# CTPLab/Tera-MIND

Hardware: AMD Instinct MI355X
Metric: denoising steps/sec on 64x64x(2 stains x 2 z) patches (interior patch-steps/s) (higher is better)
Workload: dtype f32; 1 GPU; configs[1]: b=32 images x 1 interior 64x64 patch (P=1, 128 padded + 32 collage patches/step), rna_slc=4, rna_num=229, stain=all, DDPM T=50 schedule, f32, mode A (pad+patchify -> UNet -> DDPM update); parallelism=dp1 (independent patch batches)

## Files before the change

include/teramind_hip.h:

```cpp
#ifndef TERAMIND_HIP_H
#define TERAMIND_HIP_H

#include <stddef.h>
#include <stdint.h>

#ifdef __cplusplus
extern "C" {
#endif

#define TM_ABI_VERSION 1

enum {
  TM_OK = 0,
  TM_ERR_ARG = -1,
  TM_ERR_STATE = -2,
  TM_ERR_KEY = -3,
  TM_ERR_HIP = -4,
  TM_ERR_WORKSPACE = -5
};

enum { TM_DTYPE_F32 = 0, TM_DTYPE_BF16 = 1, TM_DTYPE_F16 = 2 };
enum { TM_SAMPLE_DDPM = 0, TM_SAMPLE_DDIM = 1 };

typedef struct tm_config {
// ... 153 lines not shown
                    int64_t x_vol, int64_t y_pitch, int64_t y_depth, int64_t y_vol, const float* win_host, int n, float C1,
                    float C2, double* out, void* stream);

int tm_avgpool2_pad3(const void* src, int dtype, int V, int D, int H, int W, int64_t src_pitch, int64_t src_depth,
                     int64_t src_vol, void* dst, int64_t dst_pitch, int64_t dst_depth, int64_t dst_vol, void* stream);

typedef struct tm_prof_stats {
  uint64_t launches;
  double total_ms;
  double nominal_flops;
  double executed_flops;
  double alg_bytes;
} tm_prof_stats;
int tm_profile_enable(tm_model* m, int on);
int tm_profile_collect(tm_model* m, tm_prof_stats* out);


int tm_op_to_cb8(const void* x_ncdhw, void* y_cb8, int N, int C, int Z, int H, int W, void* stream);
int tm_op_from_cb8(const void* x_cb8, void* y_ncdhw, int N, int C, int Z, int H, int W, void* stream);

int tm_op_conv_mfma(const void* x_cb8, const void* w_host, const void* bias_host, void* y_cb8,
                    int N, int Cin, int Cout, int Z, int S, int ksize, int zmode, int up2,
                    int tile_variant, void* stream);
int tm_op_conv_mfma_res(const void* x_cb8, const void* w_host, const void* bias_host, void* y_cb8, const void* res_cb8,
                        int res_half, int N, int Cin, int Cout, int Z, int S, int ksize, int zmode, int up2,
                        int tile_variant, void* stream);

int tm_op_conv_zpair_fused_f32(const void* x_cb8, const void* w_host, const void* bias_host, const void* norm_w_host,
                               const void* scale_host, const void* shift_host, const void* res_cb8, void* a2_out,
                               void* h1_out, void* a2_sep_out, int N, int Cin, int Cout, int Z, int S, int per_image,
                               int tile_variant, void* stream);

int tm_op_conv_ups_pair_f32(const void* x_cb8, const void* w_host, const void* bias_host, void* y_cb8, int N, int Cin,
                            int Cout, int Z, int S, int tile_variant, void* stream);

int tm_op_conv_xquad_f32(const void* x_cb8, const void* w_host, const void* bias_host, void* y_cb8, const void* res_cb8,
                         int res_half, int N, int Cin, int Cout, int Z, int S, int tile_variant, void* stream);
int tm_op_conv_xquad_sched_f32(const void* x_cb8, const void* w_host, const void* bias_host, void* y_cb8, const void* res_cb8,
                               int res_half, int N, int Cin, int Cout, int Z, int S, int tile_variant, int sched, void* stream);
int tm_conv_xquad_lds_bytes(int half, int tw, int sched);
int tm_op_conv_pad1_time_sched_f32(const void* x_cb8, const void* w_host, const void* bias_host, void* y_cb8, int N, int Cin,
                                   int Cout, int S, int form, int tile_variant, int sched, int iters, float* ms_out, void* stream);
int tm_op_conv_xquad_split_f32(const void* x_cb8, const void* w_host, const void* bias_host, void* y_cb8, const void* res_cb8,
                               int res_half, int N, int Cin, int Cout, int Z, int S, int tile_variant, int sched, int ksplit,
                               void* stream);
int tm_conv_xquad_ksplit(int N, int Cin, int Cout, int S, int res_half);
int tm_op_conv_pad1_time_split_f32(const void* x_cb8, const void* w_host, const void* bias_host, void* y_cb8, int N, int Cin,
                                   int Cout, int S, int form, int tile_variant, int sched, int ksplit, int iters, float* ms_out,
                                   void* stream);

int tm_op_conv1_f32(const void* x_cb8, const void* w_host, const void* bias_host, void* y_cb8, const void* res_cb8,
                    const void* gate_cb8, int x_cbtot, int x_cb0, int gate_cbtot, int gate_cb0, int gate_half, int gelu,
                    int tile_variant, int N, int Cin, int Cout, int Z, int S, int* form_out, void* stream);
int tm_conv1_form(long vox, int ntile, int tile_variant);

int tm_conv_frag_addrs(int kernel, int half, int tw, int what, int wave, int p, int ky, int kx, int sub, int* out64);

int tm_op_conv27_bf16(const void* x_cb8, const void* w_host, const void* bias_host, void* y_cb8,
                      int N, int Cin, int Cout, int S, int dtype, int waves, const void* res_h16, void* y_h16,
                      int ups, int res_half, void* stream);
int tm_op_conv27_h16_z(const void* x_cb8, const void* w_host, const void* bias_host, void* y_cb8,
                       int N, int Cin, int Cout, int S, int dtype, int waves, const void* res_h16, void* y_h16,
                       int ups, int res_half, int Z, void* stream);

int tm_op_conv27_time(int N, int Cin, int Cout, int S, int dtype, int waves, int ups, int with_res, int fused,
                      int iters, float* ms_per_launch, void* stream);

int tm_op_conv27_fused(const void* x_cb8, const void* w_host, const void* bias_host, const void* norm_w_host,
                       const void* scale_host, const void* shift_host, void* a2_out, int N, int Cin, int Cout,
                       int S, int per_image, int dtype, int waves, void* stream);
int tm_op_conv27_fused_z(const void* x_cb8, const void* w_host, const void* bias_host, const void* norm_w_host,
                         const void* scale_host, const void* shift_host, void* a2_out, int N, int Cin, int Cout,
                         int S, int per_image, int dtype, int waves, int Z, void* stream);

int tm_op_conv1_bf16(const void* x_cb8, const void* w_host, const void* bias_host, void* y_cb8,
                     int N, int Cin, int Cout, int Z, int S, int gelu, int dtype, int waves, const void* res_h16,
                     const void* gate_h16, void* y_h16, void* stream);

int tm_op_conv1_h16_gate(const void* x_cb8, const void* w_host, const void* bias_host, void* y_cb8,
                         int N, int Cin, int Cout, int Z, int S, int gelu, int dtype, int waves, const void* res_h16,
                         const void* gate_h16, void* y_h16, int gate_half, int gate_cbtot, int gate_cb0, void* stream);

int tm_op_conv1_concat(const void* const* x_cb8, const int* cin, const int* collage, int nsrc, const void* w_host,
                       const void* bias_host, void* y_cb8, int N, int Cout, int Z, int S, int p1, int p2,
                       int dtype, int waves, void* stream);

int tm_op_prep_h16(const void* const* src_h16, const int* src_c, const int* collage, int nsrc, int N, int Z, int S,
                   int p1, int p2, int up2, const void* norm_w_dev, int c_real, int mod, const void* mod_scale,
                   const void* mod_shift, long mod_stride, int per_image, int act, int dtype, int variant,
                   void* out_h16, void* raw_h16, int iters, float* elapsed_ms, void* stream);

int tm_op_prep_f32(const void* const* src_cb8, const int* src_c, const int* collage, int nsrc, int N, int Z, int S,
                   int p1, int p2, int up2, const void* norm_w_dev, int c_real, int mod, const void* mod_scale,
                   const void* mod_shift, long mod_stride, int mod_half, int per_image, int act, int variant,
                   void* out_cb8, void* raw_cb8, int iters, float* elapsed_ms, void* stream);

int tm_op_prep_form(const void* const* src, const int* src_c, const int* collage, int nsrc, int N, int Z, int S,
                    int p1, int p2, int resample, int src_dtype, int out_dtype, const void* norm_w_dev, int c_real,
                    int mod, int mod_dtype, const void* mod_scale, const void* mod_shift, long mod_stride, int mod_half,
                    int per_image, int act, int variant, int pad_blocks, void* out, void* raw, int raw_dtype,
                    int iters, float* elapsed_ms, void* stream);

int tm_op_stem(const void* x, const void* w_host, const void* bias_host, void* y, int N, int Cin, int Cout, int Z, int S,
               int dtype, void* stream);
int tm_op_head(const void* x_cb8, const void* w_host, const void* bias_host, void* y, int N, int C, int Cout, int Z, int S,
               int dtype, void* stream);
// ... 93 lines not shown
```

tera-mind_amd/_lib.py:

```python
import ctypes as C
import os

_HERE = os.path.dirname(os.path.abspath(__file__))
LIB_PATH = os.environ.get("TM_LIB_PATH") or os.path.join(_HERE, "csrc", "libteramind_hip.so")

c_void_p, c_int, c_size_t, c_char_p, c_float = C.c_void_p, C.c_int, C.c_size_t, C.c_char_p, C.c_float
c_i64_p = C.POINTER(C.c_int64)


class TmConfig(C.Structure):
    _fields_ = [("patch_size", C.c_int32), ("rna_slc", C.c_int32), ("n_stain", C.c_int32),
                ("rna_num", C.c_int32), ("net_ch", C.c_int32), ("ch_mult", C.c_int32 * 4),
                ("embed_ch", C.c_int32), ("attn_res", C.c_int32), ("num_res_blocks", C.c_int32),
                ("vis_only", C.c_int32), ("dtype", C.c_int32)]


class TmStepCoefs(C.Structure):
    _fields_ = [("sqrt_recip_alphas_cumprod", c_float), ("sqrt_recipm1_alphas_cumprod", c_float),
                ("posterior_mean_coef1", c_float), ("posterior_mean_coef2", c_float),
                ("sigma", c_float), ("sqrt_alpha_bar_prev", c_float),
                ("sqrt_one_minus_alpha_bar_prev", c_float)]


class TmProfStats(C.Structure):
# ... 24 lines not shown
    "tm_unet_forward": (c_int, [c_void_p, c_void_p, c_void_p, c_void_p, c_int, c_int, c_int,
                                c_void_p, c_void_p, c_void_p, c_size_t, c_void_p]),
    "tm_rna_level0_bytes": (c_size_t, [c_void_p, c_int, c_int, c_int]),
    "tm_rna_level0": (c_int, [c_void_p, c_void_p, c_int, c_int, c_int, c_void_p, c_size_t, c_void_p, c_size_t, c_void_p]),
    "tm_unet_forward_level0": (c_int, [c_void_p] * 4 + [c_size_t] + [c_int] * 3 + [c_void_p] * 3 + [c_size_t, c_void_p]),
    "tm_rna_pyramid_bytes": (c_size_t, [c_void_p, c_int, c_int, c_int]),
    "tm_rna_pyramid": (c_int, [c_void_p, c_void_p, c_int, c_int, c_int, c_void_p, c_size_t, c_void_p]),
    "tm_unet_forward_rna": (c_int, [c_void_p, c_void_p, c_void_p, c_void_p, c_size_t, c_int, c_int, c_int,
                                    c_void_p, c_void_p, c_void_p, c_size_t, c_void_p]),
    "tm_sampler_step": (c_int, [C.POINTER(TmStepCoefs), c_void_p, c_void_p, c_void_p, c_void_p,
                                c_int, c_int, c_int, c_int, c_int, c_int, c_void_p]),
    "tm_pad_patchify": (c_int, [c_void_p, c_void_p, c_int, c_int, c_int, c_int, c_int, c_float, c_void_p]),
    "tm_gene_attn_workspace_bytes": (c_size_t, [c_void_p, c_int]),
    "tm_gene_attn": (c_int, [c_void_p, c_void_p, c_int, c_void_p, c_void_p, c_void_p, c_size_t, c_void_p]),
    "tm_gene_attn_readout_workspace_bytes": (c_size_t, [c_void_p, c_int, c_int]),
    "tm_gene_attn_readout": (c_int, [c_void_p, c_void_p, c_int, C.POINTER(C.c_int), c_int, c_void_p, c_void_p, c_void_p,
                                     c_size_t, c_void_p]),
    "tm_model_destroy": (c_int, [c_void_p]),
    "tm_gene_tile_dense": (c_int, [c_void_p, c_void_p, C.c_int64] + [c_int] * 6 + [c_void_p, c_void_p]),
    "tm_train_batch_images": (c_int, [c_void_p] + [c_int] * 5 + [c_void_p, c_void_p] + [c_int] * 4 + [c_void_p, c_void_p]),
    "tm_train_batch_genes": (c_int, [c_void_p, c_void_p, C.c_int64, c_void_p, c_void_p] + [c_int] * 4 + [c_void_p, c_void_p] +
                             [c_int] * 5 + [c_void_p, c_void_p]),
    "tm_blosc_decompress": (c_int, [c_void_p, c_size_t, c_void_p, c_size_t, C.POINTER(c_size_t)]),
    "tm_blosc_bound": (c_size_t, [c_size_t, c_int, c_int]),
    "tm_blosc_compress": (c_int, [c_void_p, c_size_t, c_int, c_int, c_void_p, c_size_t, c_void_p, c_void_p]),
    "tm_blosc_compress_tiles": (c_int, [c_void_p, c_int, C.c_int64] + [c_int] * 3 + [C.c_int64] * 2 + [c_void_p, c_void_p, c_int, c_void_p,
                                        C.c_int64, c_void_p, c_void_p]),
    "tm_blosc_frame_info": (c_int, [c_void_p, c_size_t, c_void_p]),
    "tm_blosc_decompress_dev": (c_int, [c_void_p, c_void_p, c_void_p, c_int, c_void_p, C.c_int64, c_void_p, c_void_p, c_void_p]),
    "tm_blosc_decompress_tiles": (c_int, [c_void_p, c_void_p, c_void_p, c_int, c_void_p, c_int] + [C.c_int64] * 3 + [c_void_p] * 3),
    "tm_u8_shrink2": (c_int, [c_void_p, c_int, c_int, C.c_int64, c_void_p, C.c_int64, c_void_p]),
    "tm_jpeg_encode_tiles": (c_int, [c_void_p, c_int, c_int, C.c_int64] + [c_int] * 3 + [c_void_p, C.c_int64] + [c_void_p] * 4),
    "tm_jpeg_tables": (c_int, [c_int, c_void_p, c_size_t, C.POINTER(c_size_t)]),
    "tm_rgb_compose": (c_int, [C.POINTER(c_void_p), c_i64_p, c_int, c_int, c_float, c_void_p] + [c_int] * 3 +
                       [c_void_p, C.c_int64, c_void_p]),
    "tm_jpeg_encode_tiles_rgb": (c_int, [C.POINTER(c_void_p), c_i64_p, c_int, c_int, c_float, c_void_p] + [c_int] * 6 +
                                 [c_void_p, C.c_int64] + [c_void_p] * 4),
    "tm_jpeg_tables_rgb": (c_int, [c_int, c_void_p, c_size_t, C.POINTER(c_size_t)]),
    "tm_heat_field": (c_int, [c_void_p] + [c_int] * 3 + [C.c_int64] * 2 + [c_int, c_int, c_float, c_int, c_int, C.POINTER(c_float),
                              c_int, c_void_p, C.c_int64, c_void_p]),
    "tm_heat_render": (c_int, [c_void_p, c_int, c_int, C.c_int64, c_int, c_float, c_float, c_void_p, c_int, c_int,
                               C.POINTER(c_void_p), c_i64_p, c_void_p, C.c_int64, c_void_p]),
    "tm_ssim_planes": (c_int, [c_void_p, c_void_p] + [c_int] * 4 + [C.c_int64] * 4 + [C.POINTER(c_float), c_int, c_float, c_float, c_void_p, c_void_p]),
    "tm_avgpool2_pad": (c_int, [c_void_p] + [c_int] * 4 + [C.c_int64] * 2 + [c_void_p] + [C.c_int64] * 2 + [c_void_p]),
    "tm_ssim_volumes": (c_int, [c_void_p, c_void_p] + [c_int] * 5 + [C.c_int64] * 6 + [C.POINTER(c_float), c_int, c_float, c_float, c_void_p, c_void_p]),
    "tm_avgpool2_pad3": (c_int, [c_void_p] + [c_int] * 5 + [C.c_int64] * 3 + [c_void_p] + [C.c_int64] * 3 + [c_void_p]),
    "tm_profile_enable": (c_int, [c_void_p, c_int]),
    "tm_profile_collect": (c_int, [c_void_p, C.POINTER(TmProfStats)]),
    "tm_op_to_cb8": (c_int, [c_void_p, c_void_p, c_int, c_int, c_int, c_int, c_int, c_void_p]),
    "tm_op_from_cb8": (c_int, [c_void_p, c_void_p, c_int, c_int, c_int, c_int, c_int, c_void_p]),
    "tm_op_conv_mfma": (c_int, [c_void_p, c_void_p, c_void_p, c_void_p] + [c_int] * 9 + [c_void_p]),
    "tm_op_conv_mfma_res": (c_int, [c_void_p, c_void_p, c_void_p, c_void_p, c_void_p] + [c_int] * 10 + [c_void_p]),
    "tm_op_conv1_f32": (c_int, [c_void_p] * 6 + [c_int] * 12 + [C.POINTER(c_int), c_void_p]),
    "tm_conv1_form": (c_int, [C.c_long, c_int, c_int]),
    "tm_conv_frag_addrs": (c_int, [c_int] * 9 + [c_void_p]),
    "tm_op_conv27_bf16": (c_int, [c_void_p, c_void_p, c_void_p, c_void_p] + [c_int] * 6 + [c_void_p] * 2 + [c_int] * 2 + [c_void_p]),
    "tm_op_conv27_fused": (c_int, [c_void_p] * 7 + [c_int] * 7 + [c_void_p]),
    "tm_op_conv27_h16_z": (c_int, [c_void_p, c_void_p, c_void_p, c_void_p] + [c_int] * 6 + [c_void_p] * 2 + [c_int] * 3 + [c_void_p]),
    "tm_op_conv27_fused_z": (c_int, [c_void_p] * 7 + [c_int] * 8 + [c_void_p]),
    "tm_op_conv_zpair_fused_f32": (c_int, [c_void_p] * 10 + [c_int] * 7 + [c_void_p]),
    "tm_op_conv_ups_pair_f32": (c_int, [c_void_p] * 4 + [c_int] * 6 + [c_void_p]),
    "tm_op_conv_xquad_f32": (c_int, [c_void_p] * 5 + [c_int] * 7 + [c_void_p]),
    "tm_op_conv_xquad_sched_f32": (c_int, [c_void_p] * 5 + [c_int] * 8 + [c_void_p]),
    "tm_conv_xquad_lds_bytes": (c_int, [c_int] * 3),
    "tm_op_conv_pad1_time_sched_f32": (c_int, [c_void_p] * 4 + [c_int] * 8 + [C.POINTER(c_float), c_void_p]),
    "tm_op_conv_xquad_split_f32": (c_int, [c_void_p] * 5 + [c_int] * 9 + [c_void_p]),
    "tm_conv_xquad_ksplit": (c_int, [c_int] * 5),
    "tm_op_conv_pad1_time_split_f32": (c_int, [c_void_p] * 4 + [c_int] * 9 + [C.POINTER(c_float), c_void_p]),
    "tm_op_conv27_time":(c_int, [c_int] * 10 + [c_void_p, c_void_p]),
    "tm_op_conv1_bf16": (c_int, [c_void_p, c_void_p, c_void_p, c_void_p] + [c_int] * 8 + [c_void_p] * 4),
    "tm_op_conv1_h16_gate": (c_int, [c_void_p, c_void_p, c_void_p, c_void_p] + [c_int] * 8 + [c_void_p] * 3 + [c_int] * 3 + [c_void_p]),
    "tm_op_conv1_concat": (c_int, [c_void_p, c_void_p, c_void_p, c_int, c_void_p, c_void_p, c_void_p] + [c_int] * 8 + [c_void_p]),
    "tm_op_prep_h16": (c_int, [c_void_p] * 3 + [c_int] * 7 + [c_void_p, c_int, c_int, c_void_p, c_void_p, C.c_long] +
                       [c_int] * 4 + [c_void_p, c_void_p, c_int, c_void_p, c_void_p]),
    "tm_op_prep_f32": (c_int, [c_void_p] * 3 + [c_int] * 7 + [c_void_p, c_int, c_int, c_void_p, c_void_p, C.c_long] +
                       [c_int] * 4 + [c_void_p, c_void_p, c_int, c_void_p, c_void_p]),
    "tm_op_prep_form": (c_int, [c_void_p] * 3 + [c_int] * 9 + [c_void_p, c_int, c_int, c_int, c_void_p, c_void_p, C.c_long] +
                        [c_int] * 5 + [c_void_p, c_void_p, c_int, c_int, c_void_p, c_void_p]),
    "tm_op_stem": (c_int, [c_void_p] * 4 + [c_int] * 6 + [c_void_p]),
    "tm_op_head": (c_int, [c_void_p] * 4 + [c_int] * 6 + [c_void_p]),
    "tm_op_time_embed": (c_int, [c_void_p] * 7 + [c_int] * 3 + [c_void_p]),
    "tm_op_emb_all": (c_int, [c_void_p] * 4 + [c_int] * 3 + [c_void_p]),
    "tm_op_prep_train": (c_int, [c_void_p] * 5 + [c_float, c_int, c_void_p] + [c_int] * 4 + [c_void_p]),
    "tm_op_prep_bwd": (c_int, [c_void_p] * 6 + [c_float, c_int] + [c_void_p] * 4 + [c_int] * 4 + [c_void_p]),
    "tm_op_prep_train_rng": (c_int, [c_void_p] * 4 + [C.c_uint64, C.c_uint, c_float, c_int, c_void_p] + [c_int] * 4 + [c_void_p]),
    "tm_op_prep_bwd_rng": (c_int, [c_void_p] * 5 + [C.c_uint64, C.c_uint, c_float, c_int] + [c_void_p] * 4 + [c_int] * 4 + [c_void_p]),
    "tm_op_dropout_mask": (c_int, [C.c_uint64, C.c_uint, c_float, c_void_p] + [c_int] * 4 + [c_void_p]),
    "tm_op_conv_dgrad": (c_int, [c_void_p, c_void_p, c_void_p] + [c_int] * 6 + [c_void_p]),
    "tm_op_conv_wgrad": (c_int, [c_void_p, c_void_p, c_void_p, c_void_p] + [c_int] * 6 + [c_void_p]),
    "tm_conv_pack_floats": (C.c_long, [c_int] * 5),
    "tm_op_conv_pack_dev": (c_int, [c_void_p, c_void_p] + [c_int] * 5 + [c_void_p]),
    "tm_op_conv_mfma_packed": (c_int, [c_void_p] * 4 + [c_int] * 6 + [c_void_p]),
    "tm_op_conv_dgrad_packed": (c_int, [c_void_p] * 3 + [c_int] * 6 + [c_void_p]),
    "tm_op_conv_wgrad_dev": (c_int, [c_void_p] * 4 + [c_int] * 7 + [c_void_p]),
    "tm_op_conv_wgrad_time": (c_int, [c_int] * 9 + [c_void_p, c_void_p]),
    "tm_op_ew": (c_int, [c_int] + [c_void_p] * 5 + [C.c_long, c_void_p]),
    "tm_op_gemm_f32": (c_int, [c_void_p] * 4 + [c_int] * 3 + [c_void_p] + [c_int] * 3 + [c_float, c_void_p]),
    "tm_op_rows": (c_int, [c_int] + [c_void_p] * 5 + [C.c_long, c_int, c_void_p]),
    "tm_op_resample": (c_int, [c_void_p, c_void_p] + [c_int] * 5 + [c_void_p]),
    "tm_op_sumsq": (c_int, [c_void_p, C.c_long, c_void_p, c_void_p]),
    "tm_op_adam": (c_int, [c_void_p] * 4 + [C.c_long] + [c_float] * 5 + [c_int, c_float, c_void_p]),
    "tm_op_rank_sum": (c_int, [c_void_p, c_void_p, c_int, C.c_long, c_void_p]),
    "tm_op_rank_sum_time": (c_int, [c_int, C.c_long, c_int, c_int, c_void_p, c_void_p]),
    "tm_op_modnorm": (c_int, [c_void_p] * 5 + [c_int] * 4 + [c_void_p]),
    "tm_op_modnorm_bwd": (c_int, [c_void_p] * 8 + [c_int] * 4 + [c_void_p]),
    "tm_op_window_attn_train": (c_int, [c_void_p] * 12 + [c_int] * 4 + [c_void_p]),
# ... 45 lines not shown
```

tera-mind_amd/csrc/tm_kernels.hip:

```cpp
#include "tm_conv_pair.h"

#include <stdlib.h>
#include <string.h>

#include <type_traits>

namespace tmk {

template <int NZI, int WM, int TW, bool UPS = false>
struct C3Geo {
  static constexpr int TW_ = TW;
  static constexpr int MV = 4 * WM * 32;
  static constexpr int TR = (MV / TW < TW) ? (MV / TW) : TW;
  static constexpr int NPB = MV / (TR * TW);
  static constexpr int HR = TR + 2, HC = TW + 2;
  static constexpr int XV = NPB * NZI * HR * HC;
  static constexpr int XPIECES = XV * 2;
  static constexpr int PX = (XPIECES + 255) / 256;
  static constexpr int TZ = UPS ? 4 : 9;
  static constexpr int NTAP = TZ * NZI;
  static constexpr int WFLOATS = NTAP * 512;
  static constexpr int WPIECES = WFLOATS / 4;
  static constexpr int PW = (WPIECES + 255) / 256;
  static constexpr int TAPS_TOTAL = (NZI == 1) ? 9 : 3 * TZ;
// ... 791 lines not shown
  for (int z = 0; z < 2; ++z)
#pragma unroll
    for (int par = 0; par < 2; ++par) {
      f32x16 o = acc[0][par] + acc[1 + z][par];
      asm volatile("" : "+v"(o));
#pragma unroll
      for (int g = 0; g < 4; ++g) {
        f32x4 v;
        v[0] = o[4 * g + 0] + bv[g][0];
        v[1] = o[4 * g + 1] + bv[g][1];
        v[2] = o[4 * g + 2] + bv[g][2];
        v[3] = o[4 * g + 3] + bv[g][3];
        if (a.flags & EPI_GELU) {
#pragma unroll
          for (int j = 0; j < 4; ++j) v[j] = gelu_tanh_hw(v[j]);
        }
        if (a.res) v = rv[z][par][g] + v;
        rv[z][par][g] = v;
        asm volatile("" : "+v"(rv[z][par][g]));
      }
    }
#pragma unroll
  for (int z = 0; z < 2; ++z)
#pragma unroll
    for (int par = 0; par < 2; ++par)
#pragma unroll
      for (int g = 0; g < 4; ++g) {
        const int cob = nt * 4 + g;
        const long uni = (long)cob * a.y_plane + z * (S * S * 8) + par * 16;
        if (cob < a.Cob && okv) *(f32x4*)(a.y + yl + uni) = rv[z][par][g];
      }
}

constexpr int XQ_ZERO_FLOATS = 4096;
__device__ float xq_zero_bias[XQ_ZERO_FLOATS];
__global__ __launch_bounds__(256) void xquad_split_reduce(const float* part, long part_stride, int ksplit, const float* bias, const float* res,
                                                          long res_nstride, float* y, long y_nstride, long per_n4, int plane4, long total4,
                                                          int flags) {
  const long i = (long)blockIdx.x * 256 + threadIdx.x;
  if (i >= total4) return;
  const long n = i / per_n4, rem = i - n * per_n4;
  const long off = n * y_nstride + rem * 4;
  f32x4 v = *(const f32x4*)(part + off);
  for (int k = 1; k < ksplit; ++k) v = v + *(const f32x4*)(part + k * part_stride + off);
  v = v + *(const f32x4*)(bias + (rem / plane4) * 8 + (rem & 1) * 4);
  if (flags & EPI_GELU) {
#pragma unroll
    for (int j = 0; j < 4; ++j) v[j] = gelu_tanh_hw(v[j]);
  }
  if (res) v = *(const f32x4*)(res + n * res_nstride + rem * 4) + v;
  *(f32x4*)(y + off) = v;
}

template <int WM, int WN>
__global__ __launch_bounds__(256, 2) void conv1_mfma(ConvArgs a) {
  constexpr int MV = 4 * WM * 32;
  constexpr int KC = 4;
  constexpr int XP = KC * MV * 2 / 256;
  constexpr int NT64 = WN / 2;
  constexpr int WP = NT64 * KC * 64 * 2 / 256;
  __shared__ __attribute__((aligned(16))) float lds[NT64 * KC * 512 + KC * MV * 8];
  float* lw = lds;
  float* lx = lds + NT64 * KC * 512;

  const int tid = threadIdx.x;
  const int lane = tid & 63, wv = tid >> 6;
  const int i32 = lane & 31, h = lane >> 5;
  const int bid = xcd_swizzle(blockIdx.x, gridDim.x);
  const int nt = bid % a.ntile;
  const int mtile = bid / a.ntile;
  const long VPN = (long)a.Z * a.S * a.S;
  const long vtot = VPN * a.N;

  long xoff[XP];
  int xkc[XP];
#pragma unroll
  for (int k = 0; k < XP; ++k) {
    const int i = tid + k * 256;
    const int half = i & 1;
    const int v = (i >> 1) % MV;
    xkc[k] = (i >> 1) / MV;
    const long vg = (long)mtile * MV + v;
    long off = -1;
    if (vg < vtot) {
      const long n = vg / VPN;
      off = n * a.x_nstride + (vg - n * VPN) * 8 + half * 4;
    }
    xoff[k] = off;
  }
  const float* wsrc = a.w + (long)nt * NT64 * a.Cbi * 512;

  int xb[WM], on[WM], ooff[WM];
#pragma unroll
  for (int mt = 0; mt < WM; ++mt) {
    const int v = (wv * WM + mt) * 32 + i32;
    xb[mt] = v * 8 + 4 * h;
    const long vg = (long)mtile * MV + v;
    if (vg < vtot) {
      const long n = vg / VPN;
      on[mt] = (int)n;
      ooff[mt] = (int)((vg - n * VPN) * 8);
    } else { on[mt] = 0; ooff[mt] = -1; }
  }
  const int wb = i32 * 8 + 4 * h;

  f32x16 acc[WN][WM];
#pragma unroll
  for (int ct = 0; ct < WN; ++ct)
#pragma unroll
    for (int mt = 0; mt < WM; ++mt)
#pragma unroll
      for (int r = 0; r < 16; ++r) acc[ct][mt][r] = 0.f;

  f32x4 xr[XP], wr[WP];
  const f32x4 zero4 = {0.f, 0.f, 0.f, 0.f};
  auto load_stage = [&](int cb0) {
#pragma unroll
    for (int k = 0; k < XP; ++k) {
      const int cb = cb0 + xkc[k];
      xr[k] = (xoff[k] >= 0 && cb < a.Cbi) ? *(const f32x4*)(a.x + (long)cb * a.x_plane + xoff[k]) : zero4;
    }
#pragma unroll
    for (int k = 0; k < WP; ++k) {
      const int i = tid + k * 256;
      const int t64 = i / (KC * 128), j = i - t64 * (KC * 128);
      const int cb = cb0 + j / 128;
      wr[k] = (cb < a.Cbi) ? *(const f32x4*)(wsrc + ((long)t64 * a.Cbi + cb0) * 512 + j * 4) : zero4;
    }
  };

  load_stage(0);
  for (int cb0 = 0; cb0 < a.Cbi; cb0 += KC) {
    __syncthreads();
#pragma unroll
    for (int k = 0; k < XP; ++k) *(f32x4*)(lx + (tid + k * 256) * 4) = xr[k];
#pragma unroll
    for (int k = 0; k < WP; ++k) *(f32x4*)(lw + (tid + k * 256) * 4) = wr[k];
    __syncthreads();
    if (cb0 + KC < a.Cbi) load_stage(cb0 + KC);
#pragma unroll
    for (int kc = 0; kc < KC; ++kc) {
      f32x4 wf[WN], xf[WM];
#pragma unroll
      for (int ct = 0; ct < WN; ++ct) wf[ct] = *(const f32x4*)(lw + (ct >> 1) * (KC * 512) + kc * 512 + (ct & 1) * 256 + wb);
#pragma unroll
      for (int mt = 0; mt < WM; ++mt) xf[mt] = *(const f32x4*)(lx + kc * MV * 8 + xb[mt]);
#pragma unroll
      for (int kk = 0; kk < 4; ++kk)
#pragma unroll
        for (int ct = 0; ct < WN; ++ct)
#pragma unroll
          for (int mt = 0; mt < WM; ++mt)
            acc[ct][mt] = __builtin_amdgcn_mfma_f32_32x32x2f32(wf[ct][kk], xf[mt][kk], acc[ct][mt], 0, 0, 0);
    }
  }
  conv_epilogue<WM, WN>(a, acc, nt, h, on, ooff, 0);
}

static bool conv_fills_chip(long vox, long tiles) { return (vox / 256) * tiles >= 512; }

int conv1_form(long vox, int ntile, int tile_variant) {
  if (tile_variant == 3) return (ntile & 1) == 0 ? 3 : 0;
  const int variant = tile_variant ? tile_variant : (conv_fills_chip(vox, ntile) ? 2 : 1);
  if (variant == 2 && (ntile & 1) == 0 && conv_fills_chip(vox, ntile / 2)) return 3;
  return variant == 2 ? 2 : 1;
}

static long xquad_large_wgs(long ovox, int ntile) { return (ovox / 1024) * 2 * ntile; }
static bool xquad_many_wgs(long ovox, int ntile, int S) { return S >= 64 && xquad_large_wgs(ovox, ntile) >= 2048; }

int xquad_ksplit(long ovox, int Cout, int Cbi, int S, bool res_half) {
  if (!xquad_split_on() || res_half || S < 8 || xquad_large_wgs(ovox, (Cout + 63) / 64) >= 256) return 1;
  const long small = (ovox + 511) / 512 * ((Cout + 31) / 32);
  return small < XQUAD_SPLIT_WGS && Cbi / 2 >= XQUAD_SPLIT_FLOOR ? 2 : 1;
}

int conv_tile(int form, long ovox, int ntile, int S, int tile_variant) {
  if (S == 4) return 1;
  if (form == CF_XQUAD)
    return tile_variant ? (tile_variant == 2 ? 2 : 1) : (xquad_large_wgs(ovox, ntile) >= 256 && !xquad_many_wgs(ovox, ntile, S) ? 2 : 1);
  const long tiles = (form == CF_ZSKIP_UPS || form == CF_PAIR_UPS) ? 4L * ntile : ntile;
  const int variant = tile_variant ? tile_variant : (conv_fills_chip(ovox, tiles) ? 2 : 1);
  return variant == 2 ? 2 : 1;
}

static bool xquad_pipe_default(bool half, int tw, bool many) {
  static const bool on = [] {
    const char* v = getenv("TM_CONV_XQUAD_PIPE");
    return !(v && atoi(v) == 0);
  }();
  return on && tw == 16 && (!half || many);
}

template <void (*KERN)(ConvArgs), class G, int BLOCK = 256>
static hipError_t launch_tiled(const ConvArgs& a, long factor, hipStream_t s) {
  static DevOnce attr_once;
  if (attr_once.need()) {
    hipError_t e = hipFuncSetAttribute((const void*)KERN, hipFuncAttributeMaxDynamicSharedMemorySize, G::LDS_BYTES);
    if (e != hipSuccess) return e;
    attr_once.mark();
  }
  const long tiles = (long)(a.S / G::TW_) * (a.S / G::TR);
  const long pgs = (a.N + G::NPB - 1) / G::NPB;
  hipLaunchKernelGGL(KERN, dim3((unsigned)(pgs * tiles * factor * a.ntile)), dim3(BLOCK), G::LDS_BYTES, s, a);
  return hipGetLastError();
}
template <int MAXTW, class F>
static hipError_t with_tile_width(int S, F f) {
  if constexpr (MAXTW >= 32)
    if (S >= 32) return f(std::integral_constant<int, 32>{});
  if (S >= 16) return f(std::integral_constant<int, 16>{});
  return f(std::integral_constant<int, 8>{});
}
template <int NZI, bool UPS>
static hipError_t launch_c3(const ConvArgs& a, bool large, hipStream_t s) {
  const long factor = UPS ? 4L * a.Z : a.Z;
  if (a.S == 4) return launch_tiled<conv3d_mfma<NZI, 1, 4, UPS>, C3Geo<NZI, 1, 4, UPS>>(a, factor, s);
  return with_tile_width<32>(a.S, [&](auto tw) {
    constexpr int TW = decltype(tw)::value;
    return large ? launch_tiled<conv3d_mfma<NZI, 2, TW, UPS>, C3Geo<NZI, 2, TW, UPS>>(a, factor, s)
                 : launch_tiled<conv3d_mfma<NZI, 1, TW, UPS>, C3Geo<NZI, 1, TW, UPS>>(a, factor, s);
  });
}

hipError_t launch_conv_mfma(const ConvLaunch& L, hipStream_t s) {
  ConvArgs a;
  a.x = L.x.p; a.x_nstride = L.x.nstride; a.x_plane = L.x.plane();
  a.w = L.w.w; a.bias = L.w.bias;
  a.y = L.y.p; a.y_nstride = L.y.nstride; a.y_plane = L.y.plane(); a.Cob = L.y.Cb;
  a.res = L.res ? L.res->p : nullptr; a.res_nstride = L.res ? L.res->nstride : 0;
  a.gate = L.gate ? L.gate->p : nullptr; a.gate_nstride = L.gate ? L.gate->nstride : 0;
  const int form = L.w.form;
  if (L.w.taps != conv_form_taps(form)) return hipErrorInvalidValue;
  if (L.gate_half) {
    int ls = 0;
    while ((1 << ls) < L.y.H) ++ls;
    if (!L.gate || form != CF_1X1 || (1 << ls) != L.y.H || L.y.H != L.y.W || ls < 1) return hipErrorInvalidValue;
    a.gate_ls = ls;
  }
  a.N = L.x.N; a.S = L.x.H; a.Z = L.x.Z; a.Cbi = L.w.Cbi; a.ntile = L.w.ntile; a.flags = L.flags;
  if (L.x.Cb != L.w.Cbi || L.x.H != L.x.W) return hipErrorInvalidValue;
  if (L.fuse_norm) {
    if (form != CF_PAIR || L.zmode != ZM_PAD1 || L.x.Z != 2 || L.w.Cout != 64 || L.w.ntile != 1 || L.res || L.gate || L.flags ||
        !L.norm_w || !L.mod_scale || !L.mod_shift || L.per_image < 1)
      return hipErrorInvalidValue;
    if (conv_tile(form, (long)L.x.N * 2 * L.x.H * L.x.H, 1, L.x.H, L.tile_variant) != 2) return hipErrorInvalidValue;
    if (!L.a2.p || L.a2.Cb != 8 || L.a2.N != L.x.N || L.a2.Z != 2 || L.a2.H != L.x.H || L.a2.W != L.x.H) return hipErrorInvalidValue;
    if (L.y.Cb != 8 || L.y.Z != 2 || L.y.H != L.x.H) return hipErrorInvalidValue;
    a.y = L.a2.p; a.y_nstride = L.a2.nstride; a.y_plane = L.a2.plane();
    a.norm_w = L.norm_w; a.mod_scale = L.mod_scale; a.mod_shift = L.mod_shift; a.mod_stride = L.mod_stride;
    a.per_image = L.per_image; a.inv_c = L.inv_c;
  }
  if (L.y.Cb > L.w.ntile * 8 || L.y.N != L.x.N) return hipErrorInvalidValue;
  const long vox = (long)a.N * a.Z * a.S * a.S;
  if (form == CF_1X1) {
    if (L.flags & EPI_UP2) return hipErrorInvalidValue;
    if (L.y.H != L.x.H || L.y.Z != L.x.Z) return hipErrorInvalidValue;
    const int form1 = conv1_form(vox, a.ntile, L.tile_variant);
    if (form1 == 3) {
      const long mt = (vox + 255) / 256;
      a.ntile /= 2;
      hipLaunchKernelGGL((conv1_mfma<2, 4>), dim3((unsigned)(mt * a.ntile)), dim3(256), 0, s, a);
    } else if (form1 == 2) {
      const long mt = (vox + 255) / 256;
      hipLaunchKernelGGL((conv1_mfma<2, 2>), dim3((unsigned)(mt * a.ntile)), dim3(256), 0, s, a);
    } else if (form1 == 1) {
      const long mt = (vox + 127) / 128;
      hipLaunchKernelGGL((conv1_mfma<1, 2>), dim3((unsigned)(mt * a.ntile)), dim3(256), 0, s, a);
    } else return hipErrorInvalidValue;
    return hipGetLastError();
  }
  const int S = a.S;
  const bool z2 = L.x.Z == 2 && L.y.Z == 2, up2 = (L.flags & EPI_UP2) != 0;
  a.Zin = L.x.Z; a.zoff = 0;
  switch (form) {
    case CF_INPLANE:
      if (L.zmode == ZM_PAD1 ? (L.x.Z != 1 || L.y.Z != 1) : (L.zmode != ZM_INPLANE || L.y.Z != L.x.Z)) return hipErrorInvalidValue;
      break;
    case CF_PLANES3:
      if (L.zmode == ZM_PAD1 ? (L.y.Z != L.x.Z || L.x.Z == 2) : (L.zmode != ZM_VALID || L.y.Z != L.x.Z - 2)) return hipErrorInvalidValue;
      if (L.zmode == ZM_PAD1) a.zoff = -1;
      break;
    case CF_ZSKIP: case CF_PAIR:
      if (L.zmode != ZM_PAD1 || !z2) return hipErrorInvalidValue;
      break;
    case CF_XQUAD:
      if (L.zmode != ZM_PAD1 || !z2 || L.x.H < 8 || up2 || L.gate) return hipErrorInvalidValue;
      break;
    case CF_ZSKIP_UPS: case CF_PAIR_UPS:
      if (L.zmode != ZM_UPS || !z2 || up2 || L.res || L.gate) return hipErrorInvalidValue;
      break;
    default: return hipErrorInvalidValue;
  }
  a.Z = L.y.Z;
  if (S != 4 && S != 8 && S != 16 && S != 32 && S != 64 && S != 128) return hipErrorInvalidValue;
  if ((up2 || L.zmode == ZM_UPS) ? (L.y.H != 2 * S) : (L.y.H != S)) return hipErrorInvalidValue;
  if (L.res_half) {
    int ls = 0;
    while ((1 << ls) < L.y.H) ++ls;
    if (!L.res || (1 << ls) != L.y.H || L.y.H != L.y.W || ls < 1 || up2) return hipErrorInvalidValue;
    a.res_ls = ls;
  }
  const bool large = conv_tile(form, (long)a.N * a.Z * a.S * a.S, a.ntile, S, L.tile_variant) == 2;
  switch (form) {
    case CF_INPLANE: return launch_c3<1, false>(a, large, s);
    case CF_PLANES3: return launch_c3<3, false>(a, large, s);
    case CF_ZSKIP: return launch_c3<2, false>(a, large, s);
    case CF_ZSKIP_UPS: return launch_c3<2, true>(a, large, s);
    case CF_PAIR:
      if (S == 4) return launch_tiled<conv3d_zpair<1, 4, false>, ZPGeo<1, 4>>(a, 1, s);
      return with_tile_width<32>(S, [&](auto tw) {
        constexpr int TW = decltype(tw)::value;
        if (L.fuse_norm) return launch_tiled<conv3d_zpair<0, TW, true>, ZPGeo<0, TW>>(a, 1, s);
        return large ? launch_tiled<conv3d_zpair<0, TW, false>, ZPGeo<0, TW>>(a, 1, s)
                     : launch_tiled<conv3d_zpair<1, TW, false>, ZPGeo<1, TW>>(a, 1, s);
      });
    case CF_PAIR_UPS:
      if (S == 4) return launch_tiled<conv3d_zpair_ups<1, 4>, ZPUGeo<1, 4>>(a, 4, s);
      return with_tile_width<32>(S, [&](auto tw) {
        constexpr int TW = decltype(tw)::value;
        return large ? launch_tiled<conv3d_zpair_ups<0, TW>, ZPUGeo<0, TW>>(a, 4, s)
// ... 1069 lines not shown
```

tera-mind_amd/csrc/tm_ops.hip:

```cpp
#include "../../include/teramind_hip.h"
#include "tm_kernels.h"

#include <algorithm>
#include <cmath>
#include <cstdint>
#include <tuple>
#include <utility>
#include <vector>
#include <string.h>

using namespace tmk;

struct DevTmp {
  std::vector<void*> ptrs;
  std::vector<hipEvent_t> events;
  hipError_t err = hipSuccess;
  const char* what = "";
  bool ordered = false;
  hipStream_t st = nullptr;
  DevTmp() = default;
  explicit DevTmp(hipStream_t stream) : ordered(true), st(stream) { keep_pool(); }
  static void keep_pool() {
    static bool done[64] = {};
    int dev = 0;
// ... 303 lines not shown
  return conv_pad1_time(x_cb8, w_host, bias_host, y_cb8, N, Cin, Cout, S, form, tile_variant, sched, 1, iters, ms_out, stream);
}
extern "C" int tm_op_conv_pad1_time_split_f32(const void* x_cb8, const void* w_host, const void* bias_host, void* y_cb8, int N, int Cin,
                                              int Cout, int S, int form, int tile_variant, int sched, int ksplit, int iters,
                                              float* ms_out, void* stream) {
  return conv_pad1_time(x_cb8, w_host, bias_host, y_cb8, N, Cin, Cout, S, form, tile_variant, sched, ksplit, iters, ms_out, stream);
}

static bool half_gate_ok(int S) { return S >= 2 && (S & (S - 1)) == 0; }

extern "C" int tm_conv1_form(long vox, int ntile, int tile_variant) { return conv1_form(vox, ntile, tile_variant); }
extern "C" int tm_conv_xquad_lds_bytes(int half, int tw, int sched) { return conv_xquad_lds_bytes(half, tw, sched); }
extern "C" int tm_conv_frag_addrs(int kernel, int half, int tw, int what, int wave, int p, int ky, int kx, int sub, int* out64) {
  return conv_frag_addrs(kernel, half, tw, what, wave, p, ky, kx, sub, out64);
}

extern "C" int tm_op_conv1_f32(const void* x_cb8, const void* w_host, const void* bias_host, void* y_cb8, const void* res_cb8,
                               const void* gate_cb8, int x_cbtot, int x_cb0, int gate_cbtot, int gate_cb0, int gate_half, int gelu,
                               int tile_variant, int N, int Cin, int Cout, int Z, int S, int* form_out, void* stream) {
  if (!x_cb8 || !w_host || !bias_host || !y_cb8) return fail(TM_ERR_ARG, "null argument");
  if (N < 1 || Cin < 1 || Cout < 1 || Z < 1 || S < 1) return fail(TM_ERR_ARG, "N, Cin, Cout, Z, S must be positive");
  const int Cbi = (Cin + 7) / 8, Cob = (Cout + 7) / 8;
  if (x_cb0 < 0 || x_cb0 + Cbi > x_cbtot)
    return fail(TM_ERR_ARG, "x slice: blocks [%d, %d) run past the %d blocks of the tensor", x_cb0, x_cb0 + Cbi, x_cbtot);
  if (gate_half && !gate_cb8) return fail(TM_ERR_ARG, "gate_half without a gate");
  if (gate_half && !half_gate_ok(S)) return fail(TM_ERR_ARG, "gate_half: S must be a power of two >= 2 (got %d)", S);
  if (gate_cb8 && (gate_cb0 < 0 || gate_cb0 + Cob > gate_cbtot))
    return fail(TM_ERR_ARG, "gate slice: blocks [%d, %d) run past the %d blocks of the tensor", gate_cb0, gate_cb0 + Cob, gate_cbtot);
  if (tile_variant < 0 || tile_variant > 3) return fail(TM_ERR_ARG, "tile_variant must be 0 (auto), 1, 2 or 3 (got %d)", tile_variant);
  ConvW cw = conv_w(CF_1X1, Cout, Cbi);
  const int form = conv1_form((long)N * Z * S * S, cw.ntile, tile_variant);
  if (!form) return fail(TM_ERR_ARG, "tile_variant 3 (128-cout tile) needs an even number of 64-cout tiles (got %d)", cw.ntile);
  if (form_out) *form_out = form;
  std::vector<float> pk(conv_pack_floats(CF_1X1, Cout, Cbi));
  conv_pack_host(CF_1X1, (const float*)w_host, Cout, &Cin, 1, pk.data());
  DevTmp tmp;
  std::tie(cw.w, cw.bias) = upload_conv(tmp, pk, bias_host, Cout);
  if (tmp.err) return tmp.report();
  ConvLaunch L;
  L.x = cb8_view(const_cast<void*>(x_cb8), N, x_cbtot * 8, Z, S, S).blocks(x_cb0, Cbi);
  L.w = cw;
  L.y = cb8_view(y_cb8, N, Cout, Z, S, S);
  L.tile_variant = tile_variant;
  L.flags = gelu ? EPI_GELU : 0;
  TV res = L.y, gate;
  if (res_cb8) { res.p = (float*)const_cast<void*>(res_cb8); L.res = &res; }
  if (gate_cb8) {
    const int Sg = gate_half ? S / 2 : S;
    gate = cb8_view(const_cast<void*>(gate_cb8), N, gate_cbtot * 8, Z, Sg, Sg).blocks(gate_cb0, Cob);
    L.gate = &gate;
    L.gate_half = gate_half ? 1 : 0;
  }
  return finish((hipStream_t)stream, launch_conv_mfma(L, (hipStream_t)stream), "conv1 (fp32)");
}

static int conv27_launch(ConvLaunchH& L, int N, int Cin, int Cout, int Z, int S, int waves, int ups, bool res, bool fused,
                         int res_half = 0) {
  if (Z < 1 || Z > 8) return fail(TM_ERR_ARG, "Z must be in 1 .. 8 (got %d)", Z);
  if (ups && Z != 2) return fail(TM_ERR_ARG, "upsampled-input form (ups): Z == 2 only (got Z = %d)", Z);
  if (res_half && Z != 2) return fail(TM_ERR_ARG, "half-resolution residual (res_half): Z == 2 only (got Z = %d)", Z);
  if (waves != 0 && waves != 4 && waves != 8 && waves != 9) return fail(TM_ERR_ARG, "waves must be 0 (auto), 4, 8 or 9 (lockstep 8-wave form)");
  if (fused && Cout != 64 && Cout != 128) return fail(TM_ERR_ARG, "fused epilogue needs Cout in {64, 128}");
  if (ups && (Cout % 128 || res)) return fail(TM_ERR_ARG, "upsampled-input form: Cout a multiple of 128, no residual");
  const int So = ups ? 2 * S : S;
  L.x = view_h16(nullptr, N, ((Cin + 7) / 8 + 1) / 2 * 16, Z, S, S);
  L.Cout = Cout; L.force_waves = waves; L.ups = ups;
  L.y = cb8_view(nullptr, N, Cout, Z, So, So);
  if (fused) { L.fuse_norm = 1; L.a2 = view_h16(nullptr, N, Cout, Z, So, So); }
  return TM_OK;
}
static int op_conv27_h16(const void* x_cb8, const void* w_host, const void* bias_host, void* y_cb8, int N, int Cin, int Cout,
                         int Z, int S, int dtype, int waves, const void* norm_w_host, const void* scale_host, const void* shift_host,
                         int per_image, void* a2_out, void* stream, const void* res_h16 = nullptr, void* y_h16 = nullptr,
                         int ups = 0, int res_half = 0) {
  if (!is_h16(dtype)) return fail(TM_ERR_ARG, "dtype must be TM_DTYPE_BF16 or TM_DTYPE_F16");
  const bool f16 = dtype == TM_DTYPE_F16, fused = norm_w_host != nullptr;
  if (fused && (!scale_host || !shift_host || !a2_out || per_image < 1))
    return fail(TM_ERR_ARG, "fused epilogue needs scale / shift / a2 and per_image >= 1");
  ConvLaunchH L;
  if (int rc = conv27_launch(L, N, Cin, Cout, Z, S, waves, ups, res_h16 != nullptr, fused, res_half)) return rc;
  hipStream_t st = (hipStream_t)stream;
  const int Cbi = (Cin + 7) / 8, nimg = (N + per_image - 1) / per_image;
  std::vector<uint16_t> pk(ups ? conv_bf16_pack_ups_elems(Cout, Cbi) : conv_bf16_pack_elems(Cout, Cbi));
  if (ups) (f16 ? conv_f16_pack_ups_host : conv_bf16_pack_ups_host)((const float*)w_host, Cout, &Cin, 1, pk.data());
  else (f16 ? conv_f16_pack_host : conv_bf16_pack_host)((const float*)w_host, Cout, &Cin, 1, pk.data());
  DevTmp tmp;
  std::tie(L.w, L.bias) = upload_conv(tmp, pk, bias_host, Cout);
  if (fused) {
    L.norm_w = tmp.alloc(Cout, (const float*)norm_w_host);
    L.mod_scale = tmp.alloc((size_t)nimg * Cout, (const float*)scale_host);
    L.mod_shift = tmp.alloc((size_t)nimg * Cout, (const float*)shift_host);
    L.mod_stride = Cout; L.per_image = per_image; L.a2.p = (uint16_t*)a2_out;
  }
  if (tmp.err) return tmp.report();
  hipError_t e = hipSuccess;
  L.x = to_h16(tmp, cb8_view(const_cast<void*>(x_cb8), N, Cin, Z, S, S), f16, true, st, e);
  L.y.p = (float*)y_cb8;
  L.res_half = res_half;
  TVH resh = as_h(L.y);
  if (res_h16) {
    resh.p = (uint16_t*)const_cast<void*>(res_h16); L.res_h = &resh;
    if (res_half) { resh.H = L.y.H / 2; resh.W = L.y.W / 2; resh.nstride = L.y.nstride / 4; }
  }
  if (y_h16) { L.y_h = (uint16_t*)y_h16; L.yh_nstride = L.y.nstride; }
  if (e == hipSuccess) e = (f16 ? launch_conv27_f16 : launch_conv27_bf16)(L, st);
  return finish(st, e, "conv27 (16-bit)");
// ... 1283 lines not shown
```

Measured before the change: 1059 interior patch-steps/s.

## Stream 1x1 conv activations straight into registers with ring prefetch and double-buffered weights

Rewrites the 1x1 conv MFMA kernel so activations are no longer staged through LDS. Each lane loads its fragment directly from global memory into a register ring R stages deep, while weights are double-buffered in LDS in fragment order, with one barrier per stage and explicit waitcnt and sched barriers. The intent is to remove the LDS round trip and one of the two syncs per K-chunk and to hide global latency. In exchange it uses more registers for the x ring, which may hurt occupancy. It also adds a host timing entry point for the 1x1 conv.

New measurement: 1063 interior patch-steps/s (median of 6 runs). About the same (+0.4%).

```diff
diff --git a/include/teramind_hip.h b/include/teramind_hip.h
--- a/include/teramind_hip.h
+++ b/include/teramind_hip.h
@@ -229,6 +229,9 @@
 int tm_op_conv1_f32(const void* x_cb8, const void* w_host, const void* bias_host, void* y_cb8, const void* res_cb8,
                     const void* gate_cb8, int x_cbtot, int x_cb0, int gate_cbtot, int gate_cb0, int gate_half, int gelu,
                     int tile_variant, int N, int Cin, int Cout, int Z, int S, int* form_out, void* stream);
+int tm_op_conv1_time_f32(const void* x_cb8, const void* w_host, const void* bias_host, void* y_cb8, const void* res_cb8,
+                         const void* gate_cb8, int x_cbtot, int x_cb0, int gate_half, int gelu, int tile_variant, int N, int Cin,
+                         int Cout, int Z, int S, int iters, float* ms_out, int* form_out, void* stream);
 int tm_conv1_form(long vox, int ntile, int tile_variant);
 
 int tm_conv_frag_addrs(int kernel, int half, int tw, int what, int wave, int p, int ky, int kx, int sub, int* out64);
diff --git a/tera-mind_amd/_lib.py b/tera-mind_amd/_lib.py
--- a/tera-mind_amd/_lib.py
+++ b/tera-mind_amd/_lib.py
@@ -100,6 +100,7 @@
     "tm_op_conv_mfma": (c_int, [c_void_p, c_void_p, c_void_p, c_void_p] + [c_int] * 9 + [c_void_p]),
     "tm_op_conv_mfma_res": (c_int, [c_void_p, c_void_p, c_void_p, c_void_p, c_void_p] + [c_int] * 10 + [c_void_p]),
     "tm_op_conv1_f32": (c_int, [c_void_p] * 6 + [c_int] * 12 + [C.POINTER(c_int), c_void_p]),
+    "tm_op_conv1_time_f32": (c_int, [c_void_p] * 6 + [c_int] * 11 + [C.POINTER(c_float), C.POINTER(c_int), c_void_p]),
     "tm_conv1_form": (c_int, [C.c_long, c_int, c_int]),
     "tm_conv_frag_addrs": (c_int, [c_int] * 9 + [c_void_p]),
     "tm_op_conv27_bf16": (c_int, [c_void_p, c_void_p, c_void_p, c_void_p] + [c_int] * 6 + [c_void_p] * 2 + [c_int] * 2 + [c_void_p]),
diff --git a/tera-mind_amd/csrc/tm_kernels.hip b/tera-mind_amd/csrc/tm_kernels.hip
--- a/tera-mind_amd/csrc/tm_kernels.hip
+++ b/tera-mind_amd/csrc/tm_kernels.hip
@@ -867,16 +867,16 @@
   *(f32x4*)(y + off) = v;
 }
 
-template <int WM, int WN>
+template <int WM, int WN, int R>
 __global__ __launch_bounds__(256, 2) void conv1_mfma(ConvArgs a) {
   constexpr int MV = 4 * WM * 32;
   constexpr int KC = 4;
-  constexpr int XP = KC * MV * 2 / 256;
   constexpr int NT64 = WN / 2;
-  constexpr int WP = NT64 * KC * 64 * 2 / 256;
-  __shared__ __attribute__((aligned(16))) float lds[NT64 * KC * 512 + KC * MV * 8];
-  float* lw = lds;
-  float* lx = lds + NT64 * KC * 512;
+  constexpr int WST = NT64 * KC * 512;
+  constexpr int WP = WST / 4 / 256;
+  constexpr int U = R / KC;
+  static_assert(R % KC == 0 && U >= 1 && U <= 4, "the ring is whole stages deep");
+  __shared__ __attribute__((aligned(16))) float lw[2 * WST];
 
   const int tid = threadIdx.x;
   const int lane = tid & 63, wv = tid >> 6;
@@ -886,38 +886,50 @@
   const int mtile = bid / a.ntile;
   const long VPN = (long)a.Z * a.S * a.S;
   const long vtot = VPN * a.N;
-
-  long xoff[XP];
-  int xkc[XP];
-#pragma unroll
-  for (int k = 0; k < XP; ++k) {
-    const int i = tid + k * 256;
-    const int half = i & 1;
-    const int v = (i >> 1) % MV;
-    xkc[k] = (i >> 1) / MV;
-    const long vg = (long)mtile * MV + v;
-    long off = -1;
-    if (vg < vtot) {
-      const long n = vg / VPN;
-      off = n * a.x_nstride + (vg - n * VPN) * 8 + half * 4;
-    }
-    xoff[k] = off;
-  }
-  const float* wsrc = a.w + (long)nt * NT64 * a.Cbi * 512;
-
-  int xb[WM], on[WM], ooff[WM];
+  const int Cbi = a.Cbi, nst = (Cbi + KC - 1) / KC;
+
+  const float* wsrc = a.w + (long)nt * NT64 * Cbi * 512;
+  const int wq = tid & 127, wh = (wq >> 3) & 1, wrow = 8 * (wq >> 4) + (wq & 7);
+  const int wsoff = wrow * 8 + wh * 4;
+  const int wdoff = (tid >> 7) * 512 + tmk::conv_frag_off(wrow, wh, 64);
+  f32x4 wr[WP];
+  auto load_w = [&](f32x4 (&dst)[WP], int st) __attribute__((always_inline)) {
+    const int s = st < nst ? st : nst - 1;
+#pragma unroll
+    for (int k = 0; k < WP; ++k) {
+      const int cb = s * KC + 2 * (k & 1) + (tid >> 7);
+      dst[k] = *(const f32x4*)(wsrc + ((long)(k >> 1) * Cbi + (cb < Cbi ? cb : Cbi - 1)) * 512 + wsoff);
+    }
+  };
+  auto store_w = [&](const f32x4 (&src)[WP], int slot) __attribute__((always_inline)) {
+#pragma unroll
+    for (int k = 0; k < WP; ++k) *(f32x4*)(lw + slot * WST + k * 1024 + wdoff) = src[k];
+  };
+  f32x4 w0[WP];
+  load_w(w0, 0);
+  load_w(wr, 1);
+
+  long xbase[WM];
+  int on[WM], ooff[WM];
 #pragma unroll
   for (int mt = 0; mt < WM; ++mt) {
-    const int v = (wv * WM + mt) * 32 + i32;
-    xb[mt] = v * 8 + 4 * h;
-    const long vg = (long)mtile * MV + v;
-    if (vg < vtot) {
-      const long n = vg / VPN;
-      on[mt] = (int)n;
-      ooff[mt] = (int)((vg - n * VPN) * 8);
-    } else { on[mt] = 0; ooff[mt] = -1; }
-  }
-  const int wb = i32 * 8 + 4 * h;
+    const long vg0 = (long)mtile * MV, vg = vg0 + (wv * WM + mt) * 32 + i32;
+    const bool ok = vg < vtot;
+    const long vc = ok ? vg : vg0;
+    const long n = vc / VPN, in = vc - n * VPN;
+    xbase[mt] = n * a.x_nstride + in * 8 + 4 * h;
+    on[mt] = ok ? (int)n : 0;
+    ooff[mt] = ok ? (int)(in * 8) : -1;
+  }
+  f32x4 xq[R][WM];
+  auto load_x = [&](int slot, int cb) __attribute__((always_inline)) {
+    const float* xp = a.x + (long)(cb < Cbi ? cb : Cbi - 1) * a.x_plane;
+#pragma unroll
+    for (int mt = 0; mt < WM; ++mt) xq[slot][mt] = *(const f32x4*)(xp + xbase[mt]);
+  };
+#pragma unroll
+  for (int r = 0; r < R - 1; ++r) load_x(r, r);
+  __builtin_amdgcn_sched_barrier(0);
 
   f32x16 acc[WN][WM];
 #pragma unroll
@@ -926,51 +938,59 @@
     for (int mt = 0; mt < WM; ++mt)
 #pragma unroll
       for (int r = 0; r < 16; ++r) acc[ct][mt][r] = 0.f;
-
-  f32x4 xr[XP], wr[WP];
-  const f32x4 zero4 = {0.f, 0.f, 0.f, 0.f};
-  auto load_stage = [&](int cb0) {
-#pragma unroll
-    for (int k = 0; k < XP; ++k) {
-      const int cb = cb0 + xkc[k];
-      xr[k] = (xoff[k] >= 0 && cb < a.Cbi) ? *(const f32x4*)(a.x + (long)cb * a.x_plane + xoff[k]) : zero4;
-    }
-#pragma unroll
-    for (int k = 0; k < WP; ++k) {
-      const int i = tid + k * 256;
-      const int t64 = i / (KC * 128), j = i - t64 * (KC * 128);
-      const int cb = cb0 + j / 128;
-      wr[k] = (cb < a.Cbi) ? *(const f32x4*)(wsrc + ((long)t64 * a.Cbi + cb0) * 512 + j * 4) : zero4;
+  store_w(w0, 0);
+
+  const int wb = tmk::conv_frag_off(i32, h, 64);
+  auto stage = [&](int st, auto u_c, auto full_c) __attribute__((always_inline)) {
+    constexpr int u = decltype(u_c)::value;
+    constexpr bool FULL = decltype(full_c)::value;
+    asm volatile("" ::: "memory");
+    __builtin_amdgcn_s_waitcnt(0xC07F);
+    __builtin_amdgcn_sched_barrier(0);
+    __builtin_amdgcn_s_barrier();
+    asm volatile("" ::: "memory");
+    __builtin_amdgcn_sched_barrier(0);
+    store_w(wr, (st + 1) & 1);
+    load_w(wr, st + 2);
+    const float* lws = lw + (st & 1) * WST + wb;
+    f32x4 wf[2][WN];
+    auto read_wf = [&](int kc) __attribute__((always_inline)) {
+#pragma unroll
+      for (int ct = 0; ct < WN; ++ct) wf[kc & 1][ct] = *(const f32x4*)(lws + ((ct >> 1) * KC + kc) * 512 + (ct & 1) * 128);
+    };
+    read_wf(0);
+#pragma unroll
+    for (int kc = 0; kc < KC; ++kc) {
+      const int cb = st * KC + kc, slot = u * KC + kc;
+      load_x((slot + R - 1) % R, cb + R - 1);
+      if (kc + 1 < KC) read_wf(kc + 1);
+      __builtin_amdgcn_sched_barrier(0);
+      if (FULL || cb < Cbi) {
+#pragma unroll
+        for (int kk = 0; kk < 4; ++kk)
+#pragma unroll
+          for (int ct = 0; ct < WN; ++ct)
+#pragma unroll
+            for (int mt = 0; mt < WM; ++mt)
+              acc[ct][mt] = __builtin_amdgcn_mfma_f32_32x32x2f32(wf[kc & 1][ct][kk], xq[slot][mt][kk], acc[ct][mt], 0, 0, 0);
+      }
+      __builtin_amdgcn_sched_barrier(0);
     }
   };
-
-  load_stage(0);
-  for (int cb0 = 0; cb0 < a.Cbi; cb0 += KC) {
-    __syncthreads();
-#pragma unroll
-    for (int k = 0; k < XP; ++k) *(f32x4*)(lx + (tid + k * 256) * 4) = xr[k];
-#pragma unroll
-    for (int k = 0; k < WP; ++k) *(f32x4*)(lw + (tid + k * 256) * 4) = wr[k];
-    __syncthreads();
-    if (cb0 + KC < a.Cbi) load_stage(cb0 + KC);
-#pragma unroll
-    for (int kc = 0; kc < KC; ++kc) {
-      f32x4 wf[WN], xf[WM];
-#pragma unroll
-      for (int ct = 0; ct < WN; ++ct) wf[ct] = *(const f32x4*)(lw + (ct >> 1) * (KC * 512) + kc * 512 + (ct & 1) * 256 + wb);
-#pragma unroll
-      for (int mt = 0; mt < WM; ++mt) xf[mt] = *(const f32x4*)(lx + kc * MV * 8 + xb[mt]);
-#pragma unroll
-      for (int kk = 0; kk < 4; ++kk)
-#pragma unroll
-        for (int ct = 0; ct < WN; ++ct)
-#pragma unroll
-          for (int mt = 0; mt < WM; ++mt)
-            acc[ct][mt] = __builtin_amdgcn_mfma_f32_32x32x2f32(wf[ct][kk], xf[mt][kk], acc[ct][mt], 0, 0, 0);
-    }
-  }
+  auto turn = [&](int st, auto full_c) __attribute__((always_inline)) {
+    constexpr bool FULL = decltype(full_c)::value;
+    stage(st, std::integral_constant<int, 0>{}, full_c);
+    if constexpr (U > 1) { if (FULL || st + 1 < nst) stage(st + 1, std::integral_constant<int, 1>{}, full_c); }
+    if constexpr (U > 2) { if (FULL || st + 2 < nst) stage(st + 2, std::integral_constant<int, 2>{}, full_c); }
+    if constexpr (U > 3) { if (FULL || st + 3 < nst) stage(st + 3, std::integral_constant<int, 3>{}, full_c); }
+  };
+  int st = 0;
+  for (; (st + U) * KC <= Cbi; st += U) turn(st, std::true_type{});
+  if (st < nst) turn(st, std::false_type{});
   conv_epilogue<WM, WN>(a, acc, nt, h, on, ooff, 0);
 }
+
+constexpr int CONV1_RING_12 = 8, CONV1_RING_22 = 8, CONV1_RING_24 = 4;
 
 static bool conv_fills_chip(long vox, long tiles) { return (vox / 256) * tiles >= 512; }
 
@@ -1075,13 +1095,13 @@
     if (form1 == 3) {
       const long mt = (vox + 255) / 256;
       a.ntile /= 2;
-      hipLaunchKernelGGL((conv1_mfma<2, 4>), dim3((unsigned)(mt * a.ntile)), dim3(256), 0, s, a);
+      hipLaunchKernelGGL((conv1_mfma<2, 4, CONV1_RING_24>), dim3((unsigned)(mt * a.ntile)), dim3(256), 0, s, a);
     } else if (form1 == 2) {
       const long mt = (vox + 255) / 256;
-      hipLaunchKernelGGL((conv1_mfma<2, 2>), dim3((unsigned)(mt * a.ntile)), dim3(256), 0, s, a);
+      hipLaunchKernelGGL((conv1_mfma<2, 2, CONV1_RING_22>), dim3((unsigned)(mt * a.ntile)), dim3(256), 0, s, a);
     } else if (form1 == 1) {
       const long mt = (vox + 127) / 128;
-      hipLaunchKernelGGL((conv1_mfma<1, 2>), dim3((unsigned)(mt * a.ntile)), dim3(256), 0, s, a);
+      hipLaunchKernelGGL((conv1_mfma<1, 2, CONV1_RING_12>), dim3((unsigned)(mt * a.ntile)), dim3(256), 0, s, a);
     } else return hipErrorInvalidValue;
     return hipGetLastError();
   }
diff --git a/tera-mind_amd/csrc/tm_ops.hip b/tera-mind_amd/csrc/tm_ops.hip
--- a/tera-mind_amd/csrc/tm_ops.hip
+++ b/tera-mind_amd/csrc/tm_ops.hip
@@ -379,6 +379,50 @@
     L.gate_half = gate_half ? 1 : 0;
   }
   return finish((hipStream_t)stream, launch_conv_mfma(L, (hipStream_t)stream), "conv1 (fp32)");
+}
+
+extern "C" int tm_op_conv1_time_f32(const void* x_cb8, const void* w_host, const void* bias_host, void* y_cb8, const void* res_cb8,
+                                    const void* gate_cb8, int x_cbtot, int x_cb0, int gate_half, int gelu, int tile_variant, int N,
+                                    int Cin, int Cout, int Z, int S, int iters, float* ms_out, int* form_out, void* stream) {
+  if (!x_cb8 || !w_host || !bias_host || !y_cb8 || !ms_out) return fail(TM_ERR_ARG, "null argument");
+  if (N < 1 || Cin < 1 || Cout < 1 || Z < 1 || S < 1 || iters < 1) return fail(TM_ERR_ARG, "N, Cin, Cout, Z, S, iters must be positive");
+  const int Cbi = (Cin + 7) / 8;
+  if (x_cb0 < 0 || x_cb0 + Cbi > x_cbtot)
+    return fail(TM_ERR_ARG, "x slice: blocks [%d, %d) run past the %d blocks of the tensor", x_cb0, x_cb0 + Cbi, x_cbtot);
+  if (gate_half && !gate_cb8) return fail(TM_ERR_ARG, "gate_half without a gate");
+  if (gate_half && !half_gate_ok(S)) return fail(TM_ERR_ARG, "gate_half: S must be a power of two >= 2 (got %d)", S);
+  if (tile_variant < 0 || tile_variant > 3) return fail(TM_ERR_ARG, "tile_variant must be 0 (auto), 1, 2 or 3 (got %d)", tile_variant);
+  ConvW cw = conv_w(CF_1X1, Cout, Cbi);
+  const int form = conv1_form((long)N * Z * S * S, cw.ntile, tile_variant);
+  if (!form) return fail(TM_ERR_ARG, "tile_variant 3 (128-cout tile) needs an even number of 64-cout tiles (got %d)", cw.ntile);
+  if (form_out) *form_out = form;
+  std::vector<float> pk(conv_pack_floats(CF_1X1, Cout, Cbi));
+  conv_pack_host(CF_1X1, (const float*)w_host, Cout, &Cin, 1, pk.data());
+  DevTmp tmp;
+  std::tie(cw.w, cw.bias) = upload_conv(tmp, pk, bias_host, Cout);
+  hipEvent_t e0 = tmp.event(), e1 = tmp.event();
+  if (tmp.err) return tmp.report();
+  ConvLaunch L;
+  L.x = cb8_view(const_cast<void*>(x_cb8), N, x_cbtot * 8, Z, S, S).blocks(x_cb0, Cbi);
+  L.w = cw;
+  L.y = cb8_view(y_cb8, N, Cout, Z, S, S);
+  L.tile_variant = tile_variant;
+  L.flags = gelu ? EPI_GELU : 0;
+  TV res = L.y, gate;
+  if (res_cb8) { res.p = (float*)const_cast<void*>(res_cb8); L.res = &res; }
+  if (gate_cb8) {
+    const int Sg = gate_half ? S / 2 : S;
+    gate = cb8_view(const_cast<void*>(gate_cb8), N, Cout, Z, Sg, Sg);
+    L.gate = &gate;
+    L.gate_half = gate_half ? 1 : 0;
+  }
+  hipStream_t st = (hipStream_t)stream;
+  HIP_TRY(hipEventRecord(e0, st));
+  for (int i = 0; i < iters; ++i) HIP_TRY(launch_conv_mfma(L, st));
+  HIP_TRY(hipEventRecord(e1, st));
+  HIP_TRY(hipEventSynchronize(e1));
+  HIP_TRY(hipEventElapsedTime(ms_out, e0, e1));
+  return finish(st, hipSuccess, "conv1_time (fp32)");
 }
 
 static int conv27_launch(ConvLaunchH& L, int N, int Cin, int Cout, int Z, int S, int waves, int ups, bool res, bool fused,
```
